# SuwoongHeo/neurecon

Measured on AMD Instinct MI355X. Metric: rays/sec (4096 rays x 128 samples, 8-layer x256 SDF MLP), higher is better.
Workload: dtype f16x3

## Files before the change

neurecon_amd/csrc/nr_capi.hip:

```cpp
#include <cmath>
#include <cstdlib>
#include <cstring>
#include <string>

#include "nr_common.h"
#include "nr_mlp.h"
#include "nr_neus.h"
#include "nr_tgemm.h"

namespace nr {

static thread_local std::string g_err;
void set_error(const std::string& msg) { g_err = msg; }

static int64_t chunk_bytes_host(int KB) { return (int64_t)(2 * KB + 1) * 1024; }

int check_sdf_desc(const NrSdfDesc* d) {
  NR_REQUIRE(d, NR_ERR_ARG, "null NrSdfDesc");
  if (d->siren) {
    NR_REQUIRE(d->D == 5 && d->W == 256 && d->skip < 0 && d->multires < 0 && d->W_geo_feat == 256,
               NR_ERR_UNSUPPORTED,
               "SIREN SDF net: only D=5, W=256, skips=[], embed_multires=-1, W_geo_feat=256 (configs/volsdf_siren.yaml)");
    NR_REQUIRE(d->precision == NR_PREC_FP32 || d->precision == NR_PREC_F16X3, NR_ERR_UNSUPPORTED,
               "SDF net: unknown precision mode");
// ... 22 lines not shown
SdfLayout sdf_layout(const NrSdfDesc& d) {
  SdfLayout L{};
  L.prec = d.precision;
  L.siren = d.siren ? 1 : 0;
  const int nops = L.siren ? kSirenOps : kSdfOps;
  const int* KB = L.siren ? kSirenKB : kSdfKB;
  const int* NBO = L.siren ? kSirenNBO : kSdfNBO;
  size_t off = 0;
  for (int i = 0; i < nops; ++i) {
    L.op_bytes[i] = (2 * KB[i] + 1) * 1024;
    L.op_off[i] = (uint32_t)off;
    off += (size_t)(NBO[i] / 2) * L.op_bytes[i];
  }
  static_assert(sdf_op_off(kSdfOps - 1) + (kSdfNBO[kSdfOps - 1] / 2) * (2 * kSdfKB[kSdfOps - 1] + 1) * 1024 > 0, "");
  L.scale_off = (uint32_t)off;
  off = align256(off + kSdfOps * 4);
  L.bound_off = (uint32_t)off;
  off = align256(off + kSdfOps * 8);
  L.w8row0_off = (uint32_t)off;
  off = align256(off + 256 * 4);
  L.misc_off = (uint32_t)off;
  off = align256(off + 16);
  L.total = (uint32_t)off;
  return L;
}

static int rad_small(const NrRadDesc& d) {
  return d.no_view_dirs ? 3 : 3 + (d.multires_view < 0 ? 3 : 3 + 6 * d.multires_view) + 3;
}

RadLayout rad_layout(const NrRadDesc& d) {
// ... 162 lines not shown
  ops[F4] = mkop(W[4], b[4], ROWS(4), 256, 0, seg(16, 0, 256), none(), seg(14, 0, n3), seg(4, n3, in0), isq2, prec, wmax + F4);
  ops[F5] = mkop(W[5], b[5], ROWS(5), 256, 0, seg(16, 0, 256), none(), seg(16, 0, 256), none(), 1.0f, prec, wmax + F5);
  ops[F6] = mkop(W[6], b[6], ROWS(6), 256, 0, seg(16, 0, 256), none(), seg(16, 0, 256), none(), 1.0f, prec, wmax + F6);
  ops[F7] = mkop(W[7], b[7], ROWS(7), 256, 0, seg(16, 0, 256), none(), seg(16, 0, 256), none(), 1.0f, prec, wmax + F7);
  ops[F8] = mkop(W[8], b[8], ROWS(8), 256, 0, seg(16, 1, 256), none(), seg(16, 0, 256), none(), 1.0f, prec, wmax + F8);
  ops[B7] = mkop(W[7], nullptr, ROWS(7), 256, 1, seg(16, 0, 256), none(), seg(16, 0, 256), none(), 1.0f, prec, wmax + B7);
  ops[B6] = mkop(W[6], nullptr, ROWS(6), 256, 1, seg(16, 0, 256), none(), seg(16, 0, 256), none(), 1.0f, prec, wmax + B6);
  ops[B5] = mkop(W[5], nullptr, ROWS(5), 256, 1, seg(16, 0, 256), none(), seg(16, 0, 256), none(), 1.0f, prec, wmax + B5);
  ops[B4] = mkop(W[4], nullptr, ROWS(4), 256, 1, seg(14, 0, n3), seg(4, n3, in0), seg(16, 0, 256), none(), isq2, prec, wmax + B4);
  ops[B3] = mkop(W[3], nullptr, ROWS(3), 256, 1, seg(16, 0, 256), none(), seg(14, 0, n3), none(), 1.0f, prec, wmax + B3);
  ops[B2] = mkop(W[2], nullptr, ROWS(2), 256, 1, seg(16, 0, 256), none(), seg(16, 0, 256), none(), 1.0f, prec, wmax + B2);
  ops[B1] = mkop(W[1], nullptr, ROWS(1), 256, 1, seg(16, 0, 256), none(), seg(16, 0, 256), none(), 1.0f, prec, wmax + B1);
  ops[B0] = mkop(W[0], nullptr, ROWS(0), in0, 1, seg(4, 0, in0), none(), seg(16, 0, 256), none(), 1.0f, prec, wmax + B0);
  float* bound = (float*)(P + L.bound_off);
  for (int i = 0; i < kSdfOps; ++i) ops[i].bound = bound + 2 * i;
  ops[F7].aux = W[8];
  char* dst[kSdfOps];
  for (int i = 0; i < kSdfOps; ++i) dst[i] = P + L.op_off[i];
  if ((rc = launch_pack_ops(ops, dst, kSdfOps, st))) return rc;
  if ((rc = launch_pack_vec(W[8], 0, 256, 256, P + L.w8row0_off, st))) return rc;
  if ((rc = launch_pack_vec(b[8], 0, 1, 4, P + L.misc_off, st))) return rc;
  return NR_OK;
}

size_t nr_mlp_workspace_bytes(int with_backward) { return with_backward ? scratch_bytes() : 0; }

int nr_sdf_forward(const NrSdfDesc* d, const void* packed, const float* pts, int64_t P, float* sdf, float* nabla,
                   float* feature, void* workspace, size_t workspace_bytes, void* stream) {
  int rc = check_sdf_desc(d);
  if (rc) return rc;
// ... 391 lines not shown
```

neurecon_amd/csrc/nr_mlp.h:

```cpp
#pragma once
#include "nr_common.h"

namespace nr {

constexpr int kWaves = 8;
constexpr int kThreads = 64 * kWaves;
constexpr int kTile = 16;
constexpr int kPointsPerWG = kTile * kWaves;
constexpr int kMaxChunkBytes = 48 * 1024;
constexpr size_t kScratchPerWG = (size_t)kWaves * 8 * 16 * 64 * 16;
constexpr int kSlabVB = 12;
constexpr int kSlab24Chunk = 2 * 64 * kSlabVB;
constexpr int kSlab24Layer = 8 * kSlab24Chunk;
constexpr int kSlabColBytes = 7 * kSlab24Layer + 16 * 64 * 16;

enum SdfOp { F0, F1, F2, F3, F4, F5, F6, F7, F8, B7, B6, B5, B4, B3, B2, B1, B0, kSdfOps };

constexpr int kSdfKB[kSdfOps] = {4, 16, 16, 16, 18, 16, 16, 16, 16, 16, 16, 16, 16, 14, 16, 16, 16};
constexpr int kSdfNBO[kSdfOps] = {16, 16, 16, 14, 16, 16, 16, 16, 16, 16, 16, 16, 18, 16, 16, 16, 4};
__host__ __device__ constexpr uint32_t sdf_op_off(int i) {
  uint32_t off = 0;
  for (int k = 0; k < i; ++k) off += (uint32_t)(kSdfNBO[k] / 2) * (2 * kSdfKB[k] + 1) * 1024;
  return off;
}

enum SirenOp { S0, S1, S2, S3, S4, SF, SB4, SB3, SB2, SB1, SB0, kSirenOps };
constexpr int kSirenKB[kSirenOps] = {4, 16, 16, 16, 16, 16, 16, 16, 16, 16, 16};
constexpr int kSirenNBO[kSirenOps] = {16, 16, 16, 16, 16, 16, 16, 16, 16, 16, 4};
static_assert(kSirenOps <= kSdfOps, "SIREN ops share SdfLayout's offset table");

struct SdfLayout {
  uint32_t op_off[kSdfOps];
  uint32_t op_bytes[kSdfOps];
  uint32_t scale_off;
  uint32_t bound_off;
  uint32_t w8row0_off;
  uint32_t misc_off;
  uint32_t total;
  int prec;
  int siren;
};

struct RadLayout {
  uint32_t op_off[5];
  uint32_t op_bytes[5];
  uint32_t head_off;
  uint32_t scale_off;
  uint32_t bound_off;
  uint32_t total;
// ... 40 lines not shown
  const float* bias;
  int64_t wn;
  int ld;
  int transpose;
  PackSeg out[2];
  PackSeg in[2];
  float scale;
  int prec;
  float* wmax;
  const float* aux;
  float* bound;
  const float* W2;
  const float* bias2;
  int64_t wn2;
  int ld2;
};

int launch_pack_op(const PackOp& op, char* dst, hipStream_t stream);
int launch_pack_ops(const PackOp* ops, char* const* dst, int nops, hipStream_t stream);
int launch_pack_vec(const float* src, int off, int nvalid, int n, char* dst, hipStream_t stream);
int launch_sdf(const SdfLayout& L, const void* packed, const float* pts, int64_t P, float* sdf, float* nabla,
               float* feature, int nfreq, void* ws, size_t ws_bytes, hipStream_t stream,
               const int* P_dev = nullptr, int P_mult = 0,
               const void* f8_alt = nullptr);
int launch_sdf_deferred(const SdfLayout& L, const void* packed, const float* pts, int64_t P, float* sdf, float* nabla,
                        int nfreq, float4* slabs, const int* tiles, const int* n_tiles, int stage, hipStream_t stream);
int launch_nerf(const NerfLayout& L, const void* packed, const float* x4, const float* vdir, int64_t vdiv,
                int64_t vmod, int64_t P, float* sigma, float* rgb, hipStream_t stream,
                const int* P_dev = nullptr);
int launch_radiance(const RadLayout& L, const void* packed, const float* x, const float* vdir, int64_t vdiv,
// ... 32 lines not shown
```

neurecon_amd/csrc/nr_mlp.hip:

```cpp
#include <algorithm>
#include <type_traits>
#include "nr_common.h"
#include "nr_mlp.h"
#include "nr_tgemm.h"

namespace nr {

using lds_ptr = __attribute__((address_space(3))) void*;

__device__ __forceinline__ void glds16(const char* gsrc, uint32_t lds_addr) {
  unsigned keep;
  asm volatile(
      "s_mov_b32 %0, m0\n\t"
      "s_mov_b32 m0, %2\n\t"
      "s_nop 0\n\t"
      "global_load_lds_dwordx4 %1, off\n\t"
      "s_mov_b32 m0, %0"
      : "=&s"(keep)
      : "v"(gsrc), "s"(lds_addr)
      : "memory");
}

__device__ __forceinline__ void glds16s(const char* sbase, uint32_t voff, uint32_t lds_addr) {
  unsigned keep;
// ... 189 lines not shown

constexpr float kSirenW0 = 30.0f;
__device__ __forceinline__ void sine_fwd(float z, float& y, float& e) {
  const float t = fmul(kSirenW0, z);
  y = sinf(t);
  e = cosf(t);
}
__device__ __forceinline__ float sine_bwd(float g, float e) { return fmul(fmul(g, e), kSirenW0); }
template <int P, int ACT>
__device__ __forceinline__ float act_bwd(float g, float e) {
  if constexpr (ACT == ACT_SINE) return sine_bwd(g, e);
  else return softplus_bwd<P>(g, e);
}

__host__ __device__ constexpr int chunk_bytes(int KB) { return (2 * KB + 1) * 1024; }

__device__ __forceinline__ f32x4 mfma16h(f16x8 a, f16x8 b, f32x4 c) {
  return __builtin_amdgcn_mfma_f32_16x16x32_f16(a, b, c, 0, 0, 0);
}
__device__ __forceinline__ f16x8 as_h8(float4 v) { return __builtin_bit_cast(f16x8, v); }

__device__ __forceinline__ float amax4(float4 v) {
  return fmaxf(fmaxf(fabsf(v.x), fabsf(v.y)), fmaxf(fabsf(v.z), fabsf(v.w)));
}
__device__ __forceinline__ float max4_groups(float m) {
  m = fmaxf(m, __uint_as_float(__builtin_amdgcn_ds_swizzle(__float_as_uint(m), 0x401F)));
  const auto r = __builtin_amdgcn_permlane32_swap(__float_as_uint(m), __float_as_uint(m), false, false);
  return fmaxf(__uint_as_float(r[0]), __uint_as_float(r[1]));
}
__device__ __forceinline__ float pow2_scale(float m) {
// ... 489 lines not shown
      }
      base = nullptr;
    }
    return issued;
  }
  __device__ __forceinline__ void put(float4* b, int cnt, bool nontemporal, bool bytes96 = false) {
    base = b;
    n = cnt;
    nt = nontemporal;
    b96 = bytes96;
  }
};

constexpr int kSlabRing = 3;
constexpr int kFwdRing = 4;
constexpr bool kSlabNT = true;
constexpr bool kFeatNT = false;

template <int CBMAX, int RING = 3, int NW = kW4>
struct WStream4 {
  static_assert(RING == 3 || RING == 4, "weight ring depth");
  static constexpr int kRingN = RING;
  static constexpr int kLd = NW == kW4 ? kLoad : NW;
  char* lds;
  char* slab;
  int cur;
  int es;
  int er;
  int prev;
  __device__ __forceinline__ static int wave_id() { return __builtin_amdgcn_readfirstlane(threadIdx.x >> 6); }
  __device__ __forceinline__ static int next3(int i) { return i == 2 ? 0 : i + 1; }
  __device__ __forceinline__ static int nextr(int i) { return i == RING - 1 ? 0 : i + 1; }
  __device__ __forceinline__ int ahead_slot() const { return cur == 0 ? RING - 1 : cur - 1; }
  template <int BYTES>
  __device__ __forceinline__ static constexpr int pieces() { return (BYTES / 1024 + kLd - 1) / kLd; }
  __device__ __forceinline__ static int loader() { return wave_id() - (NW - kLd); }
  template <int BYTES>
  __device__ __forceinline__ static int npieces() { return loader() >= 0 ? pieces<BYTES>() : 0; }
  template <int BYTES>
  __device__ __forceinline__ void dma(const char* gsrc, int slot) {
    constexpr int NB = BYTES / 1024, NPW = pieces<BYTES>();
    const int wave = loader();
    if (wave < 0) return;
    const uint32_t voff = (threadIdx.x & 63) * 16;
// ... 36 lines not shown
        glds16m(gj, voff, mj);
    }
  }
  template <int B0, int B1>
  __device__ __forceinline__ void start(const char* g0, const char* g1) {
    static_assert(RING == 3, "start: the first RING - 1 chunks");
    cur = 0;
    es = 0;
    er = 0;
    prev = 0;
    dma<B0>(g0, 0);
    dma<B1>(g1, 1);
    wait_vmcnt(npieces<B1>());
    __syncthreads();
  }
  template <int B0, int B1, int B2>
  __device__ __forceinline__ void start(const char* g0, const char* g1, const char* g2) {
    static_assert(RING == 4, "start: the first RING - 1 chunks");
    cur = 0;
    es = 0;
    er = 0;
    dma<B0>(g0, 0);
    dma<B1>(g1, 1);
    dma<B2>(g2, 2);
    prev = npieces<B2>();
    wait_vmcnt(npieces<B1>() + npieces<B2>());
    __syncthreads();
  }
  template <int BYTES>
  __device__ __forceinline__ void issue(const char* gsrc) { dma<BYTES>(gsrc, ahead_slot()); }
  __device__ __forceinline__ int stage_slab(const float4* e, int c) {
    return stage_slab(e, c, (threadIdx.x & 63) * kSlabVB);
  }
  __device__ __forceinline__ int stage_slab(const float4* e, int c, uint32_t voff) {
    const char* g = uniform_ptr((const char*)e + kNC * kSlab24Chunk * c);
    const uint32_t base =
        __builtin_amdgcn_readfirstlane(lds_u32(slab) + (uint32_t)(es * kSlab4 + wave_id() * kSlabW));
// ... 82 lines not shown
constexpr int kStampPh = 6;
__device__ unsigned long long g_nr_stamps[2048 * 8 * kStampPh];
__device__ __forceinline__ unsigned long long* stamp_lds() {
  __shared__ unsigned long long s_stamp[kW4 * kStampPh];
  return s_stamp;
}
__device__ __forceinline__ uint64_t stamp_now() { return __builtin_amdgcn_s_memtime(); }
__device__ __forceinline__ void stamp_add(int ph, uint64_t dt) {
  if ((threadIdx.x & 63) == 0) stamp_lds()[(threadIdx.x >> 6) * kStampPh + ph] += dt;
}
#define NR_STAMP(var) const uint64_t var = stamp_now()
#else
#define NR_STAMP(var)
#endif

template <int KB, int NBO, int NXT_CB, bool AUX, bool TS, class WS, class Pre, class Epi>
__device__ __forceinline__ void op4(WS& ws, const char* __restrict__ op, const char* nxt, const f16x8 (&bh)[kNC][12],
                                    const f16x8 (&bl)[kNC][12], const float (&xinv)[kNC], Pend4& pd, Pre&& pre,
                                    Epi&& epi, int lane) {
  constexpr int CB = chunk_bytes(KB);
  constexpr int NCH = NBO / 2;
  constexpr int LA = WS::kRingN - 1;
  static_assert(NCH >= 2, "the 2-ahead stream needs >= 2 chunks per op");
  const int g = lane >> 4;
  Z4 zq{};
#pragma unroll
  for (int c = 0; c < NCH; ++c) {
    const char* opc = op;
    const char* nxc = nxt;
    asm volatile("" : "+s"(opc), "+s"(nxc));
    NR_STAMP(t0);
    int npend = 0;
    if (c + LA < NCH) {
      ws.template issue<CB>(opc + (c + LA) * CB);
      npend = WS::template npieces<CB>();
    } else if (nxc) {
      ws.template issue<NXT_CB>(nxc + (c + LA - NCH) * NXT_CB);
      npend = WS::template npieces<NXT_CB>();
    }
    npend += pre(c);
    npend += pd.flush();
    NR_STAMP(t1);
    const float4* A = ws.buf();
    f32x4 acc[kNC][2] = {};
    mma4<KB / 2>(A, bh, bl, acc, lane, [&](int st) {
      if (c > 0) {
#pragma unroll
        for (int e = 0; e < 8; ++e)
          if (e * (KB / 2) / 8 == st) epi(c - 1, zq, e);
      }
    });
    NR_STAMP(t2);
    float wi = A[2 * KB * 64 + 8].x;
    if constexpr (TS) wi *= kT;
    const float4 b0 = A[2 * KB * 64 + (TS ? 24 : 0) + g], b1 = A[2 * KB * 64 + (TS ? 28 : 4) + g];
#pragma unroll
    for (int q = 0; q < kNC; ++q) {
      const float inv = xinv[q] * wi;
      zq.z[q][0] = fma4s(acc[q][0], inv, b0);
      zq.z[q][1] = fma4s(acc[q][1], inv, b1);
    }
    if constexpr (AUX) {
      zq.aux[0] = A[2 * KB * 64 + 16 + g];
      zq.aux[1] = A[2 * KB * 64 + 20 + g];
    }
#ifdef NR_EXP_STAMPS
    wait_vmcnt(npend);
    NR_STAMP(t3);
    ws.flip(npend);
    NR_STAMP(t4);
    stamp_add(0, t1 - t0);
    stamp_add(1, t2 - t1);
    stamp_add(2, t3 - t2);
    stamp_add(3, t4 - t3);
    stamp_add(4, 1);
#else
    ws.flip(npend);
#endif
  }
  pd.flush();
#pragma unroll
  for (int e = 0; e < 8; ++e) epi(NCH - 1, zq, e);
}

template <bool NABLA>
__device__ __forceinline__ void sp_pair(const Z4& zz, int q, int k, float4 (&y)[2], float4& s0, float4& s1) {
  const int o = k >> 1;
  const float4 z = zz.z[q][o];
  float4& s = o ? s1 : s0;
  if ((k & 1) == 0) softplus_pk<NABLA>(z.x, z.y, y[o].x, y[o].y, s.x, s.y);
  else softplus_pk<NABLA>(z.z, z.w, y[o].z, y[o].w, s.z, s.w);
}
__device__ __forceinline__ float4 mul4(float4 a, float4 b) { return make_float4(a.x * b.x, a.y * b.y, a.z * b.z, a.w * b.w); }
__device__ __forceinline__ uint32_t opaque_lane(int lane) {
  uint32_t l = (uint32_t)lane;
// ... 180 lines not shown
template <bool NABLA, bool FEAT, int STAGE_>
__global__ __attribute__((amdgpu_flat_work_group_size(STAGE_ == 3 ? 256 : kT4, STAGE_ == 3 ? 256 : kT4),
                          amdgpu_waves_per_eu(kWPE, kWPE)))
void sdf4_kernel(SdfKArgs a) {
  constexpr int STAGE = STAGE_ == 3 ? 0 : (STAGE_ == 4 ? 2 : STAGE_);
  constexpr bool COMPACT = STAGE_ == 4;
  constexpr int NW = STAGE_ == 3 ? 4 : kW4;
  static_assert(STAGE_ != 3 || (!NABLA && !FEAT), "narrow tiles: forward-only launches");
  static_assert(STAGE == 0 || (NABLA && !FEAT), "deferred nablas: no feature");
  constexpr int PPW = 16 * kNC * NW;
  constexpr int CB = chunk_bytes(18);
  constexpr int C16 = chunk_bytes(16), C4 = chunk_bytes(4), C14 = chunk_bytes(14), C18 = chunk_bytes(18);
  static_assert((size_t)kW4 * kNC * kSlabColBytes <= kScratchPerWG, "per-workgroup slab scratch");
  constexpr bool SLABS = NABLA && STAGE != 1;
  constexpr int RING = SLABS ? 3 : kFwdRing;
  __shared__ __attribute__((aligned(16))) char smem[RING * CB + (SLABS ? kSlabRing * kSlab4 : 0)];
  static_assert(RING * CB + (SLABS ? kSlabRing * kSlab4 : 0) <= 160 * 1024, "LDS budget");
  WStream4<CB, RING, NW> ws{smem, SLABS ? smem + RING * CB : nullptr, 0, 0, 0, 0};
  const int lane = threadIdx.x & 63, wave = __builtin_amdgcn_readfirstlane(threadIdx.x >> 6);
  const int j = lane & 15, g = lane >> 4;
  const char* W = a.packed;
  auto OP = [&](int i) {
    const char* w = W;
    asm volatile("" : "+s"(w));
    return w + sdf_op_off(i);
  };
  auto OPF8 = [&]() {
    const char* w = a.f8_alt;
    asm volatile("" : "+s"(w));
    return w ? w : OP(F8);
  };
  const float b8 = *(const float*)(W + a.L.misc_off);
  float4* escr = uniform_ptr((float4*)((char*)a.scratch + (size_t)(blockIdx.x * kW4 + wave) * (kNC * kSlabColBytes)));
  auto slab = [&](int l) {
    char* e = (char*)escr;
    asm volatile("" : "+s"(e));
    return (float4*)(e + l * kNC * kSlab24Layer);
  };

#ifdef NR_EXP_STAMPS
  if ((threadIdx.x & 63) == 0)
    for (int i = 0; i < kStampPh; ++i) stamp_lds()[wave * kStampPh + i] = 0;
#endif
  if constexpr (STAGE == 2) ws.template start<C16, C16>(OP(B7), OP(B7) + C16);
  else if constexpr (RING == 4) ws.template start<C4, C4, C4>(OP(F0), OP(F0) + C4, OP(F0) + 2 * C4);
  else ws.template start<C4, C4>(OP(F0), OP(F0) + C4);
  Pend4 pd{};
  NoPre4 nopre;
  const float kSpSlack = 0.0070f;

  const int64_t Pn = COMPACT      ? ((int64_t)(*a.n_tiles) + 15) / 16 * 16
                     : STAGE == 2 ? (int64_t)(*a.n_tiles) * kPointsPerWG / kW4
                                  : (a.P_dev ? min(a.P, (int64_t)(*a.P_dev) * a.P_mult) : a.P);
  for (int64_t base = (int64_t)blockIdx.x * PPW; base < Pn; base += (int64_t)gridDim.x * PPW) {
    const bool has_next = base + (int64_t)gridDim.x * PPW < Pn;
    int64_t p0 = base + wave * 16 * kNC;
    int plane = lane;
    uint32_t soff = 0;
    int64_t pl = 0;
    bool listed = true;
// ... 27 lines not shown
        valid[q] = listed;
        pq[q] = pl;
      } else {
        valid[q] = p < Pv;
        pq[q] = valid[q] ? p : Pv - 1;
      }
      xs[q][0] = a.pts[pq[q] * 3 + 0];
      xs[q][1] = a.pts[pq[q] * 3 + 1];
      xs[q][2] = a.pts[pq[q] * 3 + 2];
    }
    float4 E[kNC][4];
    float mE[kNC], xinv[kNC];
    f16x8 Uh[kNC][12], Ul[kNC][12], Vh[kNC][12], Vl[kNC][12];
    float mrun[kNC], m_in[kNC];
    auto next_scales = [&](int kb, float extra, const float (&floor_max)[kNC], float (&sc)[kNC]) {
      const float4 v = ws.buf()[2 * kb * 64 + 8];
#pragma unroll
      for (int q = 0; q < kNC; ++q) sc[q] = bound_scale(fmaxf(fmaf(v.y, m_in[q], v.z) + extra, floor_max[q]));
    };
    auto finish = [&](const float (&sc)[kNC], float mscale = 1.0f) {
#pragma unroll
      for (int q = 0; q < kNC; ++q) {
        m_in[q] = max4_groups(mrun[q]) * mscale;
        mrun[q] = 0.0f;
        xinv[q] = 1.0f / sc[q];
      }
    };
    float zero2[kNC];
#pragma unroll
    for (int q = 0; q < kNC; ++q) zero2[q] = 0.0f;
    if constexpr (STAGE != 2) {
#pragma unroll
    for (int q = 0; q < kNC; ++q) {
// ... 23 lines not shown
          asm volatile("global_store_dwordx4 %0, %1, %2\n\ts_nop 1" : : "v"(off), "v"(d), "s"(epark) : "memory");
        }
    }
#pragma unroll
    for (int q = 0; q < kNC; ++q) {
      mrun[q] = 0.0f;
      m_in[q] = mE[q];
    }
    auto fwd_epi = [&](f16x8(&oh)[kNC][12], f16x8(&ol)[kNC][12], const float (&sc)[kNC], float4* sl) {
      return FwdEpi4<NABLA>{oh, ol, sc, sl, mrun, pd, lane};
    };

    {
      float sc[kNC];
      next_scales(4, kSpSlack, zero2, sc);
      op4<4, 16, C16, false, true>(ws, OP(F0), OP(F1), Uh, Ul, xinv, pd, nopre, fwd_epi(Vh, Vl, sc, slab(0)), lane);
      finish(sc, kC);
    }
    {
      float sc[kNC];
      next_scales(16, kSpSlack, zero2, sc);
      op4<16, 16, C16, false, true>(ws, OP(F1), OP(F2), Vh, Vl, xinv, pd, nopre, fwd_epi(Uh, Ul, sc, slab(1)), lane);
      finish(sc, kC);
    }
    {
      float sc[kNC];
      next_scales(16, kSpSlack, zero2, sc);
      op4<16, 16, C16, false, true>(ws, OP(F2), OP(F3), Uh, Ul, xinv, pd, nopre, fwd_epi(Vh, Vl, sc, slab(2)), lane);
      finish(sc, kC);
    }
    {
      float sc[kNC];
      next_scales(16, kSpSlack, mE, sc);
      op4<16, 14, C18, false, true>(ws, OP(F3), OP(F4), Vh, Vl, xinv, pd, nopre, fwd_epi(Uh, Ul, sc, slab(3)), lane);
      if constexpr (NABLA) {
        asm volatile("s_waitcnt vmcnt(0)" ::: "memory");
#pragma unroll
        for (int q = 0; q < kNC; ++q)
#pragma unroll
          for (int b = 0; b < 4; ++b) E[q][b] = fromf(*((const gf4*)epark + ((12 + b) * kNC + q) * 64 + lane));
      }
#pragma unroll
      for (int q = 0; q < kNC; ++q) {
        split8a(E[q][0], E[q][1], sc[q], Uh[q][7], Ul[q][7]);
        split8a(E[q][2], E[q][3], sc[q], Uh[q][8], Ul[q][8]);
        mrun[q] = fmaxf(mrun[q], mE[q] * (1.0f / kC));
      }
      finish(sc, kC);
    }
    {
      float sc[kNC];
      next_scales(18, kSpSlack, zero2, sc);
      op4<18, 16, C16, false, true>(ws, OP(F4), OP(F5), Uh, Ul, xinv, pd, nopre, fwd_epi(Vh, Vl, sc, slab(4)), lane);
      finish(sc, kC);
    }
    {
      float sc[kNC];
      next_scales(16, kSpSlack, zero2, sc);
      op4<16, 16, C16, false, true>(ws, OP(F5), OP(F6), Vh, Vl, xinv, pd, nopre, fwd_epi(Uh, Ul, sc, slab(5)), lane);
      finish(sc, kC);
    }
    {
      float sc[kNC];
      next_scales(16, kSpSlack, zero2, sc);
      op4<16, 16, C16, false, true>(ws, OP(F6), OP(F7), Uh, Ul, xinv, pd, nopre, fwd_epi(Vh, Vl, sc, slab(6)), lane);
      finish(sc, kC);
    }
    float sdf_part[kNC];
#pragma unroll
    for (int q = 0; q < kNC; ++q) sdf_part[q] = 0.0f;
    {
      float sc[kNC];
      next_scales(16, kSpSlack, zero2, sc);
      F7Epi4<NABLA, FEAT> epi{Uh, Ul, sc, slab(7), mrun, sdf_part, pd, lane};
      constexpr int NXT = ((NABLA && STAGE == 0) || FEAT) ? C16 : C4;
      const char* n;
      if constexpr (FEAT) n = OPF8();
      else n = (NABLA && STAGE == 0) ? OP(B7) : (has_next ? OP(F0) : nullptr);
      op4<16, 16, NXT, true, false>(ws, OP(F7), n, Vh, Vl, xinv, pd, nopre, epi, lane);
      finish(sc);
    }
#pragma unroll
    for (int q = 0; q < kNC; ++q) {
      const float sdf = wave_sum4(sdf_part[q]) + b8;
      if (valid[q] && g == 0) a.sdf[p0 + 16 * q + j] = sdf;
    }
    if constexpr (FEAT) {
      const int64_t pf = p0 < Pn ? p0 : Pn - 1;
      float4* fb = uniform_ptr((float4*)(a.feature + pf * 256));
      uint32_t frow[kNC];
#pragma unroll
      for (int q = 0; q < kNC; ++q) frow[q] = (uint32_t)(pq[q] - pf);
      auto epi = [&](int c, const Z4& zz, int st) {
        if (st != 7) return;
#pragma unroll
        for (int q = 0; q < kNC; ++q) {
          pd.v[2 * q] = zz.z[q][0];
          pd.v[2 * q + 1] = zz.z[q][1];
          const uint32_t r = opaque_lane(frow[q] * 64 + g);
          pd.o[2 * q] = r + (2 * c) * 4;
          pd.o[2 * q + 1] = r + (2 * c + 1) * 4;
        }
        pd.put(fb, 2 * kNC, kFeatNT);
      };
      constexpr int NXT = NABLA ? C16 : C4;
      const char* n = NABLA ? OP(B7) : (has_next ? OP(F0) : nullptr);
      op4<16, 16, NXT, false, false>(ws, OPF8(), n, Uh, Ul, xinv, pd, nopre, epi, lane);
    }
    }
    if constexpr (NABLA && STAGE == 1) {
      pd.flush();
    }
    if constexpr (NABLA && STAGE != 1) {
      pd.flush();
      asm volatile("s_waitcnt vmcnt(0)" ::: "memory");
      float4* g7 = slab(7);
#pragma unroll
      for (int q = 0; q < kNC; ++q) {
        float4 G[16];
#pragma unroll
        for (int b = 0; b < 16; ++b) G[b] = fromf(*((const gf4*)g7 + (kNC * b + q) * 64 + (COMPACT ? plane : lane)));
        float m = 0.0f;
#pragma unroll
        for (int b = 0; b < 16; b += 2) m = amax8(m, G[b], G[b + 1]);
        m_in[q] = max4_groups(m);
        mrun[q] = 0.0f;
        const float sc = bound_scale(m_in[q]);
#pragma unroll
        for (int s = 0; s < 8; ++s) split8a(G[2 * s], G[2 * s + 1], sc, Uh[q][s], Ul[q][s]);
        xinv[q] = 1.0f / sc;
      }
      float4* park = slab(7);
      if constexpr (COMPACT) ws.stage_slab(slab(6), 0, soff);
      else ws.stage_slab(slab(6), 0);
      auto bwd = [&](auto kb_tag, auto nbo_tag, auto nmain_tag, auto nxt_tag, int opi, const char* nxt,
                     f16x8(&ih)[kNC][12], f16x8(&il)[kNC][12], f16x8(&oh)[kNC][12], f16x8(&ol)[kNC][12], int lcur,
                     int park_blk, int lnext) {
        constexpr int KBo = decltype(kb_tag)::value, NBOo = decltype(nbo_tag)::value;
        constexpr int NMAIN = decltype(nmain_tag)::value, NXC = decltype(nxt_tag)::value;
        float sc[kNC];
        next_scales(KBo, 0.0f, zero2, sc);
        auto pre = [&](int c) -> int {
          if constexpr (COMPACT) {
            if (2 * (c + 1) < NMAIN) return ws.stage_slab(slab(lcur), c + 1, soff);
            if (c + 1 == NBOo / 2 && lnext >= 0) return ws.stage_slab(slab(lnext), 0, soff);
          } else {
            if (2 * (c + 1) < NMAIN) return ws.stage_slab(slab(lcur), c + 1);
            if (c + 1 == NBOo / 2 && lnext >= 0) return ws.stage_slab(slab(lnext), 0);
          }
          return 0;
        };
        BwdEpi4<NMAIN, decltype(ws)> epi{oh, ol, sc, ws, park, park_blk, mrun, pd, lane, COMPACT ? plane : lane};
        op4<KBo, NBOo, NXC, false, false>(ws, OP(opi), nxt, ih, il, xinv, pd, pre, epi, lane);
        finish(sc);
      };
      using I0 = std::integral_constant<int, 0>;
      using I4 = std::integral_constant<int, 4>;
      using I14 = std::integral_constant<int, 14>;
      using I16 = std::integral_constant<int, 16>;
      using I18 = std::integral_constant<int, 18>;
      using IC16 = std::integral_constant<int, C16>;
      using IC14 = std::integral_constant<int, C14>;
      using IC4 = std::integral_constant<int, C4>;
      bwd(I16{}, I16{}, I16{}, IC16{}, B7, OP(B6), Uh, Ul, Vh, Vl, 6, 0, 5);
      bwd(I16{}, I16{}, I16{}, IC16{}, B6, OP(B5), Vh, Vl, Uh, Ul, 5, 0, 4);
      bwd(I16{}, I16{}, I16{}, IC16{}, B5, OP(B4), Uh, Ul, Vh, Vl, 4, 0, 3);
      bwd(I16{}, I18{}, I14{}, IC14{}, B4, OP(B3), Vh, Vl, Uh, Ul, 3, 0, 2);
      bwd(I14{}, I16{}, I16{}, IC16{}, B3, OP(B2), Uh, Ul, Vh, Vl, 2, 0, 1);
      bwd(I16{}, I16{}, I16{}, IC16{}, B2, OP(B1), Vh, Vl, Uh, Ul, 1, 0, 0);
      bwd(I16{}, I16{}, I16{}, IC16{}, B1, OP(B0), Uh, Ul, Vh, Vl, 0, 0, -1);
      if constexpr (STAGE == 2) bwd(I16{}, I4{}, I0{}, IC16{}, B0, has_next ? OP(B7) : nullptr, Vh, Vl, Uh, Ul, 0, 4, -1);
      else bwd(I16{}, I4{}, I0{}, IC4{}, B0, has_next ? OP(F0) : nullptr, Vh, Vl, Uh, Ul, 0, 4, -1);
      pd.flush();
      asm volatile("s_waitcnt vmcnt(0)" ::: "memory");
#pragma unroll
      for (int q = 0; q < kNC; ++q) {
        float n0 = 0.f, n1 = 0.f, n2 = 0.f;
#pragma unroll
        for (int b = 0; b < 4; ++b) {
          const float4 u = fromf(*((const gf4*)park + (kNC * b + q) * 64 + (COMPACT ? plane : lane)));
          const float4 v = fromf(*((const gf4*)park + (kNC * (4 + b) + q) * 64 + (COMPACT ? plane : lane)));
          const int f = 16 * b + 4 * g;
          embed_backward(f + 0, fadd(v.x, u.x), xs[q][0], xs[q][1], xs[q][2], a.nfreq, n0, n1, n2);
          embed_backward(f + 1, fadd(v.y, u.y), xs[q][0], xs[q][1], xs[q][2], a.nfreq, n0, n1, n2);
          embed_backward(f + 2, fadd(v.z, u.z), xs[q][0], xs[q][1], xs[q][2], a.nfreq, n0, n1, n2);
          embed_backward(f + 3, fadd(v.w, u.w), xs[q][0], xs[q][1], xs[q][2], a.nfreq, n0, n1, n2);
        }
// ... 1452 lines not shown
      const int cl = 16 * b_loc + fi;
      if (cl < op.in[s].nvalid) col = op.in[s].off + cl;
      break;
    }
    b_loc -= op.in[s].nblk;
  }
  if (row < 0 || col < 0) return 0.0f;
  if (op.W2 && ob >= op.out[0].nblk) return op.W2[(int64_t)row * op.ld2 + col] * op.scale;
  return (op.transpose ? op.W[(int64_t)col * op.ld + row] : op.W[(int64_t)row * op.ld + col]) * op.scale;
}

__device__ __forceinline__ float op_bias(const PackOp& op, int s, int row) {
  return (s == 1 && op.W2) ? op.bias2[row] : op.bias[row];
}

__device__ __forceinline__ float wscale(const PackOp& op) {
  if (op.prec != NR_PREC_F16X3) return 1.0f;
  const float m = *op.wmax;
  if (!(m > 0.0f)) return 1.0f;
  return __builtin_ldexpf(1.0f, 13 - __builtin_amdgcn_frexp_expf(m));
}

__device__ __forceinline__ void pack_word(const PackOp& op, uint32_t* __restrict__ dst, int64_t e) {
  const int KB = op.in[0].nblk + op.in[1].nblk;
  const int per_chunk = (2 * KB + 1) * 256;
  const int c = (int)(e / per_chunk);
  const int w = (int)(e - (int64_t)c * per_chunk);
  if (w >= 2 * KB * 256) {
    const int idx = w - 2 * KB * 256;
    float v = 0.0f;
    if (idx < 32 && op.bias) {
      int ob_loc = 2 * c + idx / 16;
      for (int s = 0; s < 2; ++s) {
        if (ob_loc < op.out[s].nblk) {
          const int rl = 16 * ob_loc + (idx & 15);
// ... 153 lines not shown
  }
  if (lane == 0) {
    red[0][wave] = m;
    red[1][wave] = best;
    red[2][wave] = bb;
  }
  __syncthreads();
  if (threadIdx.x == 0) {
    float a = 0.0f, b = 0.0f, c = 0.0f;
    for (int w = 0; w < 4; ++w) {
      a = fmaxf(a, red[0][w]);
      b = fmaxf(b, red[1][w]);
      c = fmaxf(c, red[2][w]);
    }
    if (op.prec == NR_PREC_F16X3) *op.wmax = a;
    if (op.bound) {
      op.bound[0] = b;
      op.bound[1] = c;
    }
  }
}

__global__ void pack_vec_kernel(const float* __restrict__ src, int off, int nvalid, int n, float* __restrict__ dst) {
  const int e = blockIdx.x * blockDim.x + threadIdx.x;
  if (e >= n) return;
  dst[e] = e < nvalid ? src[off + e] : 0.0f;
}

int launch_pack_ops(const PackOp* ops, char* const* dst, int nops, hipStream_t stream) {
  for (int b0 = 0; b0 < nops; b0 += kPackBatch) {
// ... 239 lines not shown
```

Measured before the change: 733,100.

## Stream only weights into LDS; move per-chunk bias/scale to separate table or scalars

```diff
diff --git a/neurecon_amd/csrc/nr_capi.hip b/neurecon_amd/csrc/nr_capi.hip
--- a/neurecon_amd/csrc/nr_capi.hip
+++ b/neurecon_amd/csrc/nr_capi.hip
@@ -60,7 +60,9 @@
   }
   static_assert(sdf_op_off(kSdfOps - 1) + (kSdfNBO[kSdfOps - 1] / 2) * (2 * kSdfKB[kSdfOps - 1] + 1) * 1024 > 0, "");
   L.scale_off = (uint32_t)off;
-  off = align256(off + kSdfOps * 4);
+  L.winv_off = L.scale_off + 128;
+  static_assert(kSdfOps * 4 <= 128, "max |W| and 1 / weight scale share 256 bytes");
+  off = align256(off + 128 + kSdfOps * 4);
   L.bound_off = (uint32_t)off;
   off = align256(off + kSdfOps * 8);
   L.w8row0_off = (uint32_t)off;
@@ -253,6 +255,7 @@
   ops[B0] = mkop(W[0], nullptr, ROWS(0), in0, 1, seg(4, 0, in0), none(), seg(16, 0, 256), none(), 1.0f, prec, wmax + B0);
   float* bound = (float*)(P + L.bound_off);
   for (int i = 0; i < kSdfOps; ++i) ops[i].bound = bound + 2 * i;
+  for (int i = 0; i < kSdfOps; ++i) ops[i].winv = (float*)(P + L.winv_off) + i;
   ops[F7].aux = W[8];
   char* dst[kSdfOps];
   for (int i = 0; i < kSdfOps; ++i) dst[i] = P + L.op_off[i];
diff --git a/neurecon_amd/csrc/nr_mlp.h b/neurecon_amd/csrc/nr_mlp.h
--- a/neurecon_amd/csrc/nr_mlp.h
+++ b/neurecon_amd/csrc/nr_mlp.h
@@ -33,6 +33,7 @@
   uint32_t op_off[kSdfOps];
   uint32_t op_bytes[kSdfOps];
   uint32_t scale_off;
+  uint32_t winv_off;
   uint32_t bound_off;
   uint32_t w8row0_off;
   uint32_t misc_off;
@@ -103,6 +104,7 @@
   const float* bias2;
   int64_t wn2;
   int ld2;
+  float* winv;
 };
 
 int launch_pack_op(const PackOp& op, char* dst, hipStream_t stream);
diff --git a/neurecon_amd/csrc/nr_mlp.hip b/neurecon_amd/csrc/nr_mlp.hip
--- a/neurecon_amd/csrc/nr_mlp.hip
+++ b/neurecon_amd/csrc/nr_mlp.hip
@@ -227,6 +227,7 @@
 }
 
 __host__ __device__ constexpr int chunk_bytes(int KB) { return (2 * KB + 1) * 1024; }
+__host__ __device__ constexpr int weight_bytes(int KB) { return 2 * KB * 1024; }
 
 __device__ __forceinline__ f32x4 mfma16h(f16x8 a, f16x8 b, f32x4 c) {
   return __builtin_amdgcn_mfma_f32_16x16x32_f16(a, b, c, 0, 0, 0);
@@ -746,6 +747,7 @@
 
 constexpr int kSlabRing = 3;
 constexpr int kFwdRing = 4;
+constexpr int kTabBytes = 8 * 512;
 constexpr bool kSlabNT = true;
 constexpr bool kFeatNT = false;
 
@@ -760,6 +762,8 @@
   int es;
   int er;
   int prev;
+  char* tab;
+  int tcur;
   __device__ __forceinline__ static int wave_id() { return __builtin_amdgcn_readfirstlane(threadIdx.x >> 6); }
   __device__ __forceinline__ static int next3(int i) { return i == 2 ? 0 : i + 1; }
   __device__ __forceinline__ static int nextr(int i) { return i == RING - 1 ? 0 : i + 1; }
@@ -826,13 +830,35 @@
     wait_vmcnt(npieces<B1>());
     __syncthreads();
   }
+  template <int CBN>
+  __device__ __forceinline__ void dma_tab(const char* gop, int buf) {
+    const int wave = loader();
+    if (wave < 0) return;
+    const uint32_t l = threadIdx.x & 63;
+    const uint32_t voff = (l & 31) * 16 + (l >> 5) * (uint32_t)CBN;
+    const int pair = wave & 3;
+    const char* g = uniform_ptr(gop) + (CBN - 1024) + pair * 2 * CBN;
+    const uint32_t base =
+        __builtin_amdgcn_readfirstlane(lds_u32(tab) + (uint32_t)(buf * kTabBytes) + (uint32_t)(pair * 1024));
+    glds16m(g, voff, base);
+  }
+  __device__ __forceinline__ static int ntab() { return loader() >= 0 ? 1 : 0; }
+  __device__ __forceinline__ const float4* tab_entry(int c) const {
+    uint32_t off = tcur * kTabBytes;
+    asm volatile("" : "+s"(off));
+    return (const float4*)(tab + off + c * 512);
+  }
   template <int B0, int B1, int B2>
-  __device__ __forceinline__ void start(const char* g0, const char* g1, const char* g2) {
+  __device__ __forceinline__ void start(const char* g0, const char* g1, const char* g2) { start<B0, B1, B2, 0>(g0, g1, g2, nullptr); }
+  template <int B0, int B1, int B2, int CBT>
+  __device__ __forceinline__ void start(const char* g0, const char* g1, const char* g2, const char* gt) {
     static_assert(RING == 4, "start: the first RING - 1 chunks");
     cur = 0;
     es = 0;
     er = 0;
+    tcur = 0;
     dma<B0>(g0, 0);
+    if constexpr (CBT != 0) dma_tab<CBT>(gt, 0);
     dma<B1>(g1, 1);
     dma<B2>(g2, 2);
     prev = npieces<B2>();
@@ -945,12 +971,19 @@
 #define NR_STAMP(var)
 #endif
 
-template <int KB, int NBO, int NXT_CB, bool AUX, bool TS, class WS, class Pre, class Epi>
+enum { kSlot = 0, kLean = 1, kTab = 2 };
+template <int KB, int NBO, int NXT_CB, bool AUX, bool TS, int MODE = kSlot, int NXT_MODE = kSlot, class WS,
+          class Pre, class Epi>
 __device__ __forceinline__ void op4(WS& ws, const char* __restrict__ op, const char* nxt, const f16x8 (&bh)[kNC][12],
                                     const f16x8 (&bl)[kNC][12], const float (&xinv)[kNC], Pend4& pd, Pre&& pre,
-                                    Epi&& epi, int lane) {
+                                    Epi&& epi, int lane, float winv = 0.0f) {
   constexpr int CB = chunk_bytes(KB);
+  constexpr bool LEAN = MODE == kLean;
+  constexpr int FB = MODE != kSlot ? weight_bytes(KB) : CB;
+  constexpr int NXT_FB = NXT_MODE != kSlot ? NXT_CB - 1024 : NXT_CB;
+  static_assert(!LEAN || (!AUX && !TS), "lean ops carry no per-row data");
   constexpr int NCH = NBO / 2;
+  static_assert(MODE != kTab || NCH * 512 <= kTabBytes, "bias table entries");
   constexpr int LA = WS::kRingN - 1;
   static_assert(NCH >= 2, "the 2-ahead stream needs >= 2 chunks per op");
   const int g = lane >> 4;
@@ -963,11 +996,17 @@
     NR_STAMP(t0);
     int npend = 0;
     if (c + LA < NCH) {
-      ws.template issue<CB>(opc + (c + LA) * CB);
-      npend = WS::template npieces<CB>();
+      ws.template issue<FB>(opc + (c + LA) * CB);
+      npend = WS::template npieces<FB>();
     } else if (nxc) {
-      ws.template issue<NXT_CB>(nxc + (c + LA - NCH) * NXT_CB);
-      npend = WS::template npieces<NXT_CB>();
+      ws.template issue<NXT_FB>(nxc + (c + LA - NCH) * NXT_CB);
+      npend = WS::template npieces<NXT_FB>();
+      if constexpr (NXT_MODE == kTab) {
+        if (c + LA == NCH) {
+          ws.template dma_tab<NXT_CB>(nxc, ws.tcur ^ 1);
+          npend += WS::ntab();
+        }
+      }
     }
     npend += pre(c);
     npend += pd.flush();
@@ -982,9 +1021,18 @@
       }
     });
     NR_STAMP(t2);
-    float wi = A[2 * KB * 64 + 8].x;
-    if constexpr (TS) wi *= kT;
-    const float4 b0 = A[2 * KB * 64 + (TS ? 24 : 0) + g], b1 = A[2 * KB * 64 + (TS ? 28 : 4) + g];
+    float wi;
+    float4 b0, b1;
+    if constexpr (LEAN) {
+      wi = winv;
+      b0 = b1 = make_float4(0.f, 0.f, 0.f, 0.f);
+    } else {
+      const float4* S = MODE == kTab ? ws.tab_entry(c) : A + 2 * KB * 64;
+      wi = S[8].x;
+      if constexpr (TS) wi *= kT;
+      b0 = S[(TS ? 24 : 0) + g];
+      b1 = S[(TS ? 28 : 4) + g];
+    }
 #pragma unroll
     for (int q = 0; q < kNC; ++q) {
       const float inv = xinv[q] * wi;
@@ -992,8 +1040,9 @@
       zq.z[q][1] = fma4s(acc[q][1], inv, b1);
     }
     if constexpr (AUX) {
-      zq.aux[0] = A[2 * KB * 64 + 16 + g];
-      zq.aux[1] = A[2 * KB * 64 + 20 + g];
+      const float4* S = MODE == kTab ? ws.tab_entry(c) : A + 2 * KB * 64;
+      zq.aux[0] = S[16 + g];
+      zq.aux[1] = S[20 + g];
     }
 #ifdef NR_EXP_STAMPS
     wait_vmcnt(npend);
@@ -1010,6 +1059,7 @@
 #endif
   }
   pd.flush();
+  if constexpr (MODE == kTab) ws.tcur ^= 1;
 #pragma unroll
   for (int e = 0; e < 8; ++e) epi(NCH - 1, zq, e);
 }
@@ -1220,9 +1270,13 @@
   static_assert((size_t)kW4 * kNC * kSlabColBytes <= kScratchPerWG, "per-workgroup slab scratch");
   constexpr bool SLABS = NABLA && STAGE != 1;
   constexpr int RING = SLABS ? 3 : kFwdRing;
-  __shared__ __attribute__((aligned(16))) char smem[RING * CB + (SLABS ? kSlabRing * kSlab4 : 0)];
-  static_assert(RING * CB + (SLABS ? kSlabRing * kSlab4 : 0) <= 160 * 1024, "LDS budget");
-  WStream4<CB, RING, NW> ws{smem, SLABS ? smem + RING * CB : nullptr, 0, 0, 0, 0};
+  constexpr bool TABF = !SLABS;
+  constexpr int FM = TABF ? kTab : kSlot;
+  constexpr int LDSB = RING * CB + (SLABS ? kSlabRing * kSlab4 : 0) + (TABF ? 2 * kTabBytes : 0);
+  __shared__ __attribute__((aligned(16))) char smem[LDSB];
+  static_assert(LDSB <= 160 * 1024, "LDS budget");
+  static_assert(!TABF || RING * CB + 2 * kTabBytes == LDSB, "the bias table follows the weight ring");
+  WStream4<CB, RING, NW> ws{smem, SLABS ? smem + RING * CB : nullptr, 0, 0, 0, 0, TABF ? smem + RING * CB : nullptr, 0};
   const int lane = threadIdx.x & 63, wave = __builtin_amdgcn_readfirstlane(threadIdx.x >> 6);
   const int j = lane & 15, g = lane >> 4;
   const char* W = a.packed;
@@ -1248,8 +1302,11 @@
   if ((threadIdx.x & 63) == 0)
     for (int i = 0; i < kStampPh; ++i) stamp_lds()[wave * kStampPh + i] = 0;
 #endif
-  if constexpr (STAGE == 2) ws.template start<C16, C16>(OP(B7), OP(B7) + C16);
-  else if constexpr (RING == 4) ws.template start<C4, C4, C4>(OP(F0), OP(F0) + C4, OP(F0) + 2 * C4);
+  constexpr bool LEANR = STAGE == 2 || (NABLA && FEAT);
+  constexpr int W16 = weight_bytes(16);
+  if constexpr (STAGE == 2) ws.template start<W16, W16>(OP(B7), OP(B7) + C16);
+  else if constexpr (TABF)
+    ws.template start<weight_bytes(4), weight_bytes(4), weight_bytes(4), C4>(OP(F0), OP(F0) + C4, OP(F0) + 2 * C4, OP(F0));
   else ws.template start<C4, C4>(OP(F0), OP(F0) + C4);
   Pend4 pd{};
   NoPre4 nopre;
@@ -1307,9 +1364,19 @@
     f16x8 Uh[kNC][12], Ul[kNC][12], Vh[kNC][12], Vl[kNC][12];
     float mrun[kNC], m_in[kNC];
     auto next_scales = [&](int kb, float extra, const float (&floor_max)[kNC], float (&sc)[kNC]) {
-      const float4 v = ws.buf()[2 * kb * 64 + 8];
+      const float4 v = TABF ? ws.tab_entry(0)[8] : ws.buf()[2 * kb * 64 + 8];
 #pragma unroll
       for (int q = 0; q < kNC; ++q) sc[q] = bound_scale(fmaxf(fmaf(v.y, m_in[q], v.z) + extra, floor_max[q]));
+    };
+    struct OpScal {
+      float winv, R, B;
+    };
+    auto op_scal = [&](int opi) {
+      const char* w = W;
+      asm volatile("" : "+s"(w));
+      typedef __attribute__((address_space(4))) const float cfloat;
+      cfloat* rb = (cfloat*)(w + a.L.bound_off + 8 * opi);
+      return OpScal{*(cfloat*)(w + a.L.winv_off + 4 * opi), rb[0], rb[1]};
     };
     auto finish = [&](const float (&sc)[kNC], float mscale = 1.0f) {
 #pragma unroll
@@ -1363,25 +1430,25 @@
     {
       float sc[kNC];
       next_scales(4, kSpSlack, zero2, sc);
-      op4<4, 16, C16, false, true>(ws, OP(F0), OP(F1), Uh, Ul, xinv, pd, nopre, fwd_epi(Vh, Vl, sc, slab(0)), lane);
+      op4<4, 16, C16, false, true, FM, FM>(ws, OP(F0), OP(F1), Uh, Ul, xinv, pd, nopre, fwd_epi(Vh, Vl, sc, slab(0)), lane);
       finish(sc, kC);
     }
     {
       float sc[kNC];
       next_scales(16, kSpSlack, zero2, sc);
-      op4<16, 16, C16, false, true>(ws, OP(F1), OP(F2), Vh, Vl, xinv, pd, nopre, fwd_epi(Uh, Ul, sc, slab(1)), lane);
+      op4<16, 16, C16, false, true, FM, FM>(ws, OP(F1), OP(F2), Vh, Vl, xinv, pd, nopre, fwd_epi(Uh, Ul, sc, slab(1)), lane);
       finish(sc, kC);
     }
     {
       float sc[kNC];
       next_scales(16, kSpSlack, zero2, sc);
-      op4<16, 16, C16, false, true>(ws, OP(F2), OP(F3), Uh, Ul, xinv, pd, nopre, fwd_epi(Vh, Vl, sc, slab(2)), lane);
+      op4<16, 16, C16, false, true, FM, FM>(ws, OP(F2), OP(F3), Uh, Ul, xinv, pd, nopre, fwd_epi(Vh, Vl, sc, slab(2)), lane);
       finish(sc, kC);
     }
     {
       float sc[kNC];
       next_scales(16, kSpSlack, mE, sc);
-      op4<16, 14, C18, false, true>(ws, OP(F3), OP(F4), Vh, Vl, xinv, pd, nopre, fwd_epi(Uh, Ul, sc, slab(3)), lane);
+      op4<16, 14, C18, false, true, FM, FM>(ws, OP(F3), OP(F4), Vh, Vl, xinv, pd, nopre, fwd_epi(Uh, Ul, sc, slab(3)), lane);
       if constexpr (NABLA) {
         asm volatile("s_waitcnt vmcnt(0)" ::: "memory");
 #pragma unroll
@@ -1400,19 +1467,19 @@
     {
       float sc[kNC];
       next_scales(18, kSpSlack, zero2, sc);
-      op4<18, 16, C16, false, true>(ws, OP(F4), OP(F5), Uh, Ul, xinv, pd, nopre, fwd_epi(Vh, Vl, sc, slab(4)), lane);
+      op4<18, 16, C16, false, true, FM, FM>(ws, OP(F4), OP(F5), Uh, Ul, xinv, pd, nopre, fwd_epi(Vh, Vl, sc, slab(4)), lane);
       finish(sc, kC);
     }
     {
       float sc[kNC];
       next_scales(16, kSpSlack, zero2, sc);
-      op4<16, 16, C16, false, true>(ws, OP(F5), OP(F6), Vh, Vl, xinv, pd, nopre, fwd_epi(Uh, Ul, sc, slab(5)), lane);
+      op4<16, 16, C16, false, true, FM, FM>(ws, OP(F5), OP(F6), Vh, Vl, xinv, pd, nopre, fwd_epi(Uh, Ul, sc, slab(5)), lane);
       finish(sc, kC);
     }
     {
       float sc[kNC];
       next_scales(16, kSpSlack, zero2, sc);
-      op4<16, 16, C16, false, true>(ws, OP(F6), OP(F7), Uh, Ul, xinv, pd, nopre, fwd_epi(Vh, Vl, sc, slab(6)), lane);
+      op4<16, 16, C16, false, true, FM, FM>(ws, OP(F6), OP(F7), Uh, Ul, xinv, pd, nopre, fwd_epi(Vh, Vl, sc, slab(6)), lane);
       finish(sc, kC);
     }
     float sdf_part[kNC];
@@ -1426,7 +1493,7 @@
       const char* n;
       if constexpr (FEAT) n = OPF8();
       else n = (NABLA && STAGE == 0) ? OP(B7) : (has_next ? OP(F0) : nullptr);
-      op4<16, 16, NXT, true, false>(ws, OP(F7), n, Vh, Vl, xinv, pd, nopre, epi, lane);
+      op4<16, 16, NXT, true, false, FM, FM>(ws, OP(F7), n, Vh, Vl, xinv, pd, nopre, epi, lane);
       finish(sc);
     }
 #pragma unroll
@@ -1454,7 +1521,8 @@
       };
       constexpr int NXT = NABLA ? C16 : C4;
       const char* n = NABLA ? OP(B7) : (has_next ? OP(F0) : nullptr);
-      op4<16, 16, NXT, false, false>(ws, OPF8(), n, Uh, Ul, xinv, pd, nopre, epi, lane);
+      op4<16, 16, NXT, false, false, FM, NABLA ? (LEANR ? kLean : kSlot) : FM>(ws, OPF8(), n, Uh, Ul, xinv, pd, nopre, epi,
+                                                                               lane);
     }
     }
     if constexpr (NABLA && STAGE == 1) {
@@ -1463,6 +1531,8 @@
     if constexpr (NABLA && STAGE != 1) {
       pd.flush();
       asm volatile("s_waitcnt vmcnt(0)" ::: "memory");
+      OpScal osn{};
+      if constexpr (LEANR) osn = op_scal(B7);
       float4* g7 = slab(7);
 #pragma unroll
       for (int q = 0; q < kNC; ++q) {
@@ -1482,13 +1552,21 @@
       float4* park = slab(7);
       if constexpr (COMPACT) ws.stage_slab(slab(6), 0, soff);
       else ws.stage_slab(slab(6), 0);
-      auto bwd = [&](auto kb_tag, auto nbo_tag, auto nmain_tag, auto nxt_tag, int opi, const char* nxt,
+      auto bwd = [&](auto kb_tag, auto nbo_tag, auto nmain_tag, auto nxt_tag, auto nxl_tag, int opi, const char* nxt,
                      f16x8(&ih)[kNC][12], f16x8(&il)[kNC][12], f16x8(&oh)[kNC][12], f16x8(&ol)[kNC][12], int lcur,
                      int park_blk, int lnext) {
         constexpr int KBo = decltype(kb_tag)::value, NBOo = decltype(nbo_tag)::value;
         constexpr int NMAIN = decltype(nmain_tag)::value, NXC = decltype(nxt_tag)::value;
+        constexpr bool NXL = decltype(nxl_tag)::value;
+        const OpScal os = osn;
         float sc[kNC];
-        next_scales(KBo, 0.0f, zero2, sc);
+        if constexpr (LEANR) {
+          if (opi != B0) osn = op_scal(opi + 1);
+#pragma unroll
+          for (int q = 0; q < kNC; ++q) sc[q] = bound_scale(fmaxf(fmaf(os.R, m_in[q], os.B) + 0.0f, zero2[q]));
+        } else {
+          next_scales(KBo, 0.0f, zero2, sc);
+        }
         auto pre = [&](int c) -> int {
           if constexpr (COMPACT) {
             if (2 * (c + 1) < NMAIN) return ws.stage_slab(slab(lcur), c + 1, soff);
@@ -1500,7 +1578,8 @@
           return 0;
         };
         BwdEpi4<NMAIN, decltype(ws)> epi{oh, ol, sc, ws, park, park_blk, mrun, pd, lane, COMPACT ? plane : lane};
-        op4<KBo, NBOo, NXC, false, false>(ws, OP(opi), nxt, ih, il, xinv, pd, pre, epi, lane);
+        constexpr int RM = LEANR ? kLean : kSlot, RMN = (LEANR && NXL) ? kLean : kSlot;
+        op4<KBo, NBOo, NXC, false, false, RM, RMN>(ws, OP(opi), nxt, ih, il, xinv, pd, pre, epi, lane, os.winv);
         finish(sc);
       };
       using I0 = std::integral_constant<int, 0>;
@@ -1511,15 +1590,17 @@
       using IC16 = std::integral_constant<int, C16>;
       using IC14 = std::integral_constant<int, C14>;
       using IC4 = std::integral_constant<int, C4>;
-      bwd(I16{}, I16{}, I16{}, IC16{}, B7, OP(B6), Uh, Ul, Vh, Vl, 6, 0, 5);
-      bwd(I16{}, I16{}, I16{}, IC16{}, B6, OP(B5), Vh, Vl, Uh, Ul, 5, 0, 4);
-      bwd(I16{}, I16{}, I16{}, IC16{}, B5, OP(B4), Uh, Ul, Vh, Vl, 4, 0, 3);
-      bwd(I16{}, I18{}, I14{}, IC14{}, B4, OP(B3), Vh, Vl, Uh, Ul, 3, 0, 2);
-      bwd(I14{}, I16{}, I16{}, IC16{}, B3, OP(B2), Uh, Ul, Vh, Vl, 2, 0, 1);
-      bwd(I16{}, I16{}, I16{}, IC16{}, B2, OP(B1), Vh, Vl, Uh, Ul, 1, 0, 0);
-      bwd(I16{}, I16{}, I16{}, IC16{}, B1, OP(B0), Uh, Ul, Vh, Vl, 0, 0, -1);
-      if constexpr (STAGE == 2) bwd(I16{}, I4{}, I0{}, IC16{}, B0, has_next ? OP(B7) : nullptr, Vh, Vl, Uh, Ul, 0, 4, -1);
-      else bwd(I16{}, I4{}, I0{}, IC4{}, B0, has_next ? OP(F0) : nullptr, Vh, Vl, Uh, Ul, 0, 4, -1);
+      using LeanNext = std::true_type;
+      using SlotNext = std::false_type;
+      bwd(I16{}, I16{}, I16{}, IC16{}, LeanNext{}, B7, OP(B6), Uh, Ul, Vh, Vl, 6, 0, 5);
+      bwd(I16{}, I16{}, I16{}, IC16{}, LeanNext{}, B6, OP(B5), Vh, Vl, Uh, Ul, 5, 0, 4);
+      bwd(I16{}, I16{}, I16{}, IC16{}, LeanNext{}, B5, OP(B4), Uh, Ul, Vh, Vl, 4, 0, 3);
+      bwd(I16{}, I18{}, I14{}, IC14{}, LeanNext{}, B4, OP(B3), Vh, Vl, Uh, Ul, 3, 0, 2);
+      bwd(I14{}, I16{}, I16{}, IC16{}, LeanNext{}, B3, OP(B2), Uh, Ul, Vh, Vl, 2, 0, 1);
+      bwd(I16{}, I16{}, I16{}, IC16{}, LeanNext{}, B2, OP(B1), Vh, Vl, Uh, Ul, 1, 0, 0);
+      bwd(I16{}, I16{}, I16{}, IC16{}, LeanNext{}, B1, OP(B0), Uh, Ul, Vh, Vl, 0, 0, -1);
+      if constexpr (STAGE == 2) bwd(I16{}, I4{}, I0{}, IC16{}, LeanNext{}, B0, has_next ? OP(B7) : nullptr, Vh, Vl, Uh, Ul, 0, 4, -1);
+      else bwd(I16{}, I4{}, I0{}, IC4{}, SlotNext{}, B0, has_next ? OP(F0) : nullptr, Vh, Vl, Uh, Ul, 0, 4, -1);
       pd.flush();
       asm volatile("s_waitcnt vmcnt(0)" ::: "memory");
 #pragma unroll
@@ -3002,11 +3083,13 @@
   return (s == 1 && op.W2) ? op.bias2[row] : op.bias[row];
 }
 
-__device__ __forceinline__ float wscale(const PackOp& op) {
-  if (op.prec != NR_PREC_F16X3) return 1.0f;
-  const float m = *op.wmax;
+__device__ __forceinline__ float wscale_of(int prec, float m) {
+  if (prec != NR_PREC_F16X3) return 1.0f;
   if (!(m > 0.0f)) return 1.0f;
   return __builtin_ldexpf(1.0f, 13 - __builtin_amdgcn_frexp_expf(m));
+}
+__device__ __forceinline__ float wscale(const PackOp& op) {
+  return wscale_of(op.prec, op.prec == NR_PREC_F16X3 ? *op.wmax : 0.0f);
 }
 
 __device__ __forceinline__ void pack_word(const PackOp& op, uint32_t* __restrict__ dst, int64_t e) {
@@ -3190,6 +3273,7 @@
       c = fmaxf(c, red[2][w]);
     }
     if (op.prec == NR_PREC_F16X3) *op.wmax = a;
+    if (op.winv) *op.winv = 1.0f / wscale_of(op.prec, a);
     if (op.bound) {
       op.bound[0] = b;
       op.bound[1] = c;
```

Result: faster. 746,400 (median of 6 runs) (+1.8%).
